# kwea123/nerf_pl

Hardware: AMD Instinct MI355X
Metric: rays/sec (64+128 samples), full training step: render_rays fwd + MSE + bwd + grad all-reduce + Adam (higher is better)
Workload: dtype bf16

## Files before the change

### nerf_pl_amd/csrc/mlp_bwd_dw.hip

```cpp
#include "mlp_device.h"
#include "mlp_bwd_dw.h"

namespace nerfhip {

#if NERFHIP_DW_PROBE
__device__ unsigned g_dw_probe[1024 * 8 * 8];
#endif

constexpr int kDwRingKiB = 160, kDwMaxDepth = 12;
constexpr int kDwFragRing = 5, kDwFragRing2D = 4;

template <int PREC> struct DwTraits;
template <> struct DwTraits<NERFHIP_BF16> {
    static constexpr int SPP = 1;
    static constexpr int RING_BYTES = kDwRingKiB * 1024;
    static constexpr int DEPTH = 0, STAGE_BYTES = 0;
};
template <> struct DwTraits<NERFHIP_F32> {
    static constexpr int SPP = 2;
    static constexpr int DEPTH = 2;
    static constexpr int MAXP = 72;
    static constexpr int STAGE_BYTES = MAXP * kPieceBytes;
    static constexpr int RING_BYTES = DEPTH * STAGE_BYTES;
};

template <int PREC> NH_HD constexpr int dw_depth(int pieces) {
    if (PREC != NERFHIP_BF16) return DwTraits<PREC>::DEPTH;
    const int d = DwTraits<PREC>::RING_BYTES / (pieces * kPieceBytes);
    return d > kDwMaxDepth ? kDwMaxDepth : d;
}

__device__ __forceinline__ void dw_bias_sum(const bf16x8& a, float& s0, float& s1) {
    const bf16x2 one = {(__bf16)1.0f, (__bf16)1.0f};
    s0 = __builtin_amdgcn_fdot2_f32_bf16(bf16x2{a[0], a[1]}, one, s0, false);
    s1 = __builtin_amdgcn_fdot2_f32_bf16(bf16x2{a[2], a[3]}, one, s1, false);
    s0 = __builtin_amdgcn_fdot2_f32_bf16(bf16x2{a[4], a[5]}, one, s0, false);
    s1 = __builtin_amdgcn_fdot2_f32_bf16(bf16x2{a[6], a[7]}, one, s1, false);
}

template <int F, int SLABS>
__device__ __forceinline__ bf16x8 dw_encode_slab(const float (&v)[3], int h, int ks) {
    constexpr int NPAIR = 3 * (F / 2);
    constexpr float kInv2PiHi = 0.15915494f, kInv2PiLo = 6.4206297e-9f;
    float rh[3], rl[3];
#pragma unroll
    for (int c = 0; c < 3; ++c) {
        const float vs = h ? 2.0f * v[c] : v[c];
        rh[c] = vs * kInv2PiHi;
        rl[c] = __builtin_fmaf(vs, kInv2PiHi, -rh[c]) + vs * kInv2PiLo;
    }
    bf16x8 out;
#pragma unroll
    for (int q = 0; q < 4; ++q) {
        const int p = 4 * ks + q;
        float s, co;
        if (p < NPAIR) {
            const int i = p / 3, c = p - 3 * i;
            const float sc = (float)(1 << (2 * i));
            const float rhc = c == 0 ? rh[0] : (c == 1 ? rh[1] : rh[2]), rlc = c == 0 ? rl[0] : (c == 1 ? rl[1] : rl[2]);
            const float t = __builtin_amdgcn_fractf(rhc * sc) + rlc * sc;
            s = __builtin_amdgcn_sinf(t);
            co = __builtin_amdgcn_cosf(t);
        } else {
            const int tail = 2 * (p - NPAIR);
            s = (tail == 0) ? (h ? v[2] : v[0]) : 0.0f;
            co = (tail == 0) ? (h ? 0.0f : v[1]) : 0.0f;
        }
        out[2 * q] = (__bf16)s;
        out[2 * q + 1] = (__bf16)co;
    }
    return out;
}

template <int PREC>
__global__ __launch_bounds__(512, 2)
void mlp_bwd_dw_kernel(DwJobTable jobs, float* __restrict__ slabs) {
    constexpr int SPP = DwTraits<PREC>::SPP;
    constexpr int SLAB_BYTES = SPP * kPieceBytes;
    constexpr int IL = act_il(PREC);
    constexpr int RING_BYTES = DwTraits<PREC>::RING_BYTES;
    __shared__ __attribute__((aligned(1024))) char ring[RING_BYTES];

    const int lane = threadIdx.x & 63;
    const int wave = __builtin_amdgcn_readfirstlane((int)(threadIdx.x >> 6));
    int jid = 0;
#pragma unroll
    for (int j = 1; j < kDwMaxJobs; ++j) jid += ((int)blockIdx.x >= jobs.soff[j]) ? 1 : 0;
    const int nsplit = jobs.nsplit[jid], split = (int)blockIdx.x - jobs.soff[jid];
    const DwJob jb = jobs.job[jid];
    const int64_t ntiles = jobs.ntiles[jid];
    const uint8_t* __restrict__ acts_base = jobs.acts[jid];
    const uint8_t* __restrict__ dys_base = jobs.dys[jid];
    [[maybe_unused]] const float* __restrict__ enc_rays = jobs.enc_rays[jid / kNumDwJobs];
    [[maybe_unused]] const float* __restrict__ enc_z = jobs.enc_z[jid / kNumDwJobs];
    [[maybe_unused]] const int enc_tpr = jobs.enc_tpr[jid / kNumDwJobs];
    const int n_ot = jb.dy_slabs / 2;
    const int n_xs = jb.x1_slabs + jb.x2_slabs;
    const int n_xt = n_xs / 2;
    const int64_t per = (ntiles + nsplit - 1) / nsplit;
    const int64_t t_first = (int64_t)split * per;
    const int64_t my_tiles = (t_first >= ntiles) ? 0 : ((ntiles - t_first < per) ? ntiles - t_first : per);
    const unsigned lds_base = (unsigned)(uintptr_t)ring;

    const int dma_off_even = (PREC == NERFHIP_BF16) ? ((lane & 1) * 32 + (lane >> 1)) * 16 : lane * 16;
    const int dma_off_odd = (PREC == NERFHIP_BF16) ? ((lane & 1) * 32 + ((lane ^ 8) >> 1)) * 16 : lane * 16;

    f32x16 acc[kDwMaxXTiles];
#pragma unroll
    for (int x = 0; x < kDwMaxXTiles; ++x)
#pragma unroll
        for (int r = 0; r < 16; ++r) acc[x][r] = 0.0f;
    float dbacc = 0.0f;
    [[maybe_unused]] float dbacc2 = 0.0f;

    const int grp = lane >> 4, c = lane & 15;
    const int tr_off = (grp & 1) * SLAB_BYTES + (2 * (8 * (grp >> 1) + (c >> 2)) + ((c & 3) & 1)) * 16 + ((c & 3) >> 1) * 8;
    const int tr_s0 = (grp & 1) ? 128 : 0, tr_s1 = 128 - tr_s0;
    [[maybe_unused]] auto load_frag = [&](const char* pb, int q) { return load_frag_tr16(pb, tr_off, tr_s0, tr_s1, q); };
    const int m32 = lane & 31, kk = lane >> 5;
    const int f32_off = (m32 >> 4) * SLAB_BYTES + (slab_nat_h(m32 & 15) * 32) * 32 + slab_nat_j(m32 & 15) * 4;
#if NERFHIP_DW_PROBE
    unsigned pr_wait = 0, pr_bar = 0, pr_issue = 0, pr_comp = 0, pr_depth = 0;
    const uint64_t pr_t00 = __builtin_amdgcn_s_memrealtime();
#endif

    auto run = [&](auto nxt_c, auto nsl_c, auto regen_c) {
        constexpr int NXT = decltype(nxt_c)::value, NSL = decltype(nsl_c)::value;
        constexpr bool REGEN = decltype(regen_c)::value;
        static_assert(!REGEN || (PREC == NERFHIP_BF16 && (NXT == 2 || NXT == 9 || NXT == 10)), "classes with an encoding section");
        constexpr int ENC = REGEN ? (NXT == 9 ? kDirSlabs : kXyzSlabs) : 0;
        constexpr int DYS = NXT == 9 ? 8 : 16;
        constexpr bool FOLD = NXT == 9 && NSL == kDwFoldStageSlabs;
        constexpr bool SPLIT2D = (PREC == NERFHIP_BF16) && (NXT == 8 || NXT == 10) && (NSL - 2 * NXT >= 16);
        constexpr int NP = NSL * SPP;
        constexpr int NPD = NP - ENC;
        constexpr int LPWD = (NPD + 7) / 8;
        constexpr int LPW = LPWD + (REGEN ? 1 : 0);
        constexpr int STAGE = (PREC == NERFHIP_BF16) ? NP * kPieceBytes : DwTraits<PREC>::STAGE_BYTES;
        constexpr int ZSLOT = 256;
        constexpr int D0 = dw_depth<PREC>(NP);
        constexpr int D = (REGEN && D0 * (STAGE + ZSLOT) > RING_BYTES) ? D0 - 1 : D0;
        static_assert(D >= 2 && D * (STAGE + (REGEN ? ZSLOT : 0)) <= RING_BYTES, "ring stages of this job class");
        static_assert((D - 2) * LPW <= 63, "counted vmcnt");
#if NERFHIP_DW_PROBE
        pr_depth = D;
#endif
        int s_issue = 0, s_use = 0;
        const uint8_t* abase = nullptr;
        const uint8_t* dbase = nullptr;
        unsigned slot = 0;
        auto stage_tile = [&](int64_t it) {
            int64_t T = t_first + (it < my_tiles ? it : my_tiles - 1);
            if (T >= ntiles) T = ntiles - 1;
            return T;
        };
        const float* zsrc = nullptr;
        unsigned zslot = 0;
        int z_issue = 0, g_slot = 0;
        const unsigned lds_z = lds_base + (unsigned)(D * STAGE);
        auto next_z = [&](int64_t st) {
            zsrc = enc_z + stage_tile(st) * 32 + (lane & 31);
            zslot = (unsigned)__builtin_amdgcn_readfirstlane((int)(lds_z + (unsigned)(z_issue * ZSLOT)));
            z_issue = (z_issue + 1 == D) ? 0 : z_issue + 1;
        };
        auto next_stage = [&](int64_t it) {
            const int64_t T = stage_tile(it);
            abase = acts_base + tile_block_off(T, act_tile_bytes(PREC), IL);
            dbase = dys_base + tile_block_off(T, kDySlabs * 64 * (16 * SPP), IL);
            slot = lds_base + (unsigned)(s_issue * STAGE);
            s_issue = (s_issue + 1 == D) ? 0 : s_issue + 1;
            if constexpr (REGEN) next_z(it + 1);
        };
        float ray_next[6] = {0.f, 0.f, 0.f, 0.f, 0.f, 0.f};
        auto load_ray = [&](int64_t st) {
            if (wave < ENC) {
                const unsigned r = (unsigned)__builtin_amdgcn_readfirstlane((int)((unsigned)stage_tile(st) / (unsigned)enc_tpr));
                typedef const float __attribute__((address_space(4))) * ConstF;
                const ConstF rp = (ConstF)(uintptr_t)(enc_rays + (size_t)r * 8);
#pragma unroll
                for (int c = 0; c < 6; ++c) ray_next[c] = rp[c];
            }
        };
        auto gen_stage = [&](int64_t st) {
            if (wave < ENC) {
                const int n = lane & 31, h = lane >> 5;
                bf16x8 e;
                if constexpr (NXT == 9) {
                    const float dv[3] = {ray_next[3], ray_next[4], ray_next[5]};
                    e = dw_encode_slab<4, kDirSlabs>(dv, h, wave);
                } else {
                    const float zv = *reinterpret_cast<const float*>(ring + D * STAGE + g_slot * ZSLOT + n * 4);
                    float xv[3];
#pragma unroll
                    for (int c = 0; c < 3; ++c) xv[c] = nh_add(ray_next[c], nh_mul(ray_next[3 + c], zv));
                    e = dw_encode_slab<10, kXyzSlabs>(xv, h, wave);
                }
                const int unit = (2 * n + h) ^ ((wave & 1) ? 8 : 0);
                *reinterpret_cast<bf16x8*>(ring + g_slot * STAGE + (DYS + wave) * SLAB_BYTES + unit * 16) = e;
            }
            g_slot = (g_slot + 1 == D) ? 0 : g_slot + 1;
            load_ray(st + 1);
        };
        constexpr int REM = NPD % 8;
        constexpr bool SHARE_LAST = (PREC == NERFHIP_BF16) && (REM == 4 || REM == 2);
        const int share_piece = NPD - REM + (SHARE_LAST ? (wave * REM) / 8 : 0);
        const unsigned long long share_mask = REM == 4 ? (0xffffffffull << (32 * (wave & 1))) : (0xffffull << (16 * (wave & 3)));
        auto issue_piece = [&](int i) {
            if constexpr (REGEN) {
                if (i == LPW - 1) {
                    glds4(zsrc, zslot);
                    return;
                }
            }
            int pi = wave + 8 * i;
            const bool shared = SHARE_LAST && i == LPWD - 1;
            if (shared) pi = share_piece;
            if (pi >= NPD) pi = NPD - 1;
            if (REGEN && pi >= DYS) pi += ENC;
            const int sl = pi / SPP, sub = pi % SPP;
            const uint8_t* src;
            if (FOLD && sl >= kDwFoldSigmaSlab) src = dbase + (size_t)(kDySigma + sl - kDwFoldSigmaSlab) * 64 * (16 * SPP) * IL;
            else if (sl < jb.dy_slabs) src = dbase + (size_t)(jb.dy_off + sl) * 64 * (16 * SPP) * IL;
            else if (sl < jb.dy_slabs + jb.x1_slabs) src = abase + (size_t)(jb.x1_off + sl - jb.dy_slabs) * 64 * (16 * SPP) * IL;
            else src = abase + (size_t)(jb.x2_off + sl - jb.dy_slabs - jb.x1_slabs) * 64 * (16 * SPP) * IL;
            const uint8_t* g = src + (size_t)sub * kPieceBytes + ((sl & 1) ? dma_off_odd : dma_off_even);
            const unsigned dst = (unsigned)__builtin_amdgcn_readfirstlane((int)(slot + (unsigned)(pi * kPieceBytes)));
            if (shared) glds16_nt_masked(g, dst, share_mask);
            else glds16_nt(g, dst);
        };
        auto issue_stage = [&](int64_t it) {
            next_stage(it);
#pragma unroll
            for (int i = 0; i < LPW; ++i) issue_piece(i);
        };
        constexpr bool SPREAD = (PREC == NERFHIP_BF16);
        constexpr int DMA_STEP = (2 * NXT) / LPW > 0 ? (2 * NXT) / LPW : 1;
        if constexpr (REGEN) {
            next_z(0);
            glds4(zsrc, zslot);
            load_ray(0);
        }
#pragma unroll
        for (int s = 0; s < D - 1; ++s) issue_stage(s);
        if constexpr (REGEN) {
            wait_vm<(D - 1) * LPW>();
            gen_stage(0);
        }
        for (int64_t it = 0; it < my_tiles; ++it) {
#if NERFHIP_DW_PROBE
            const unsigned t0 = shader_cycles();
            wait_vm<(PREC == NERFHIP_BF16) ? (D - 2) * LPW : 0>();
            const unsigned t1 = shader_cycles();
            asm volatile("s_barrier" ::: "memory");
            const unsigned t2 = shader_cycles();
            pr_wait += (t1 - t0) & 0xffffffffu;
            pr_bar += (t2 - t1) & 0xffffffffu;
#else
            wait_vm_barrier<(PREC == NERFHIP_BF16) ? (D - 2) * LPW : 0>();
#endif
            if (SPREAD && (SPLIT2D || wave < n_ot)) next_stage(it + D - 1);
            else issue_stage(it + D - 1);
#if NERFHIP_DW_PROBE
            const unsigned t3 = shader_cycles();
            pr_issue += (t3 - t2) & 0xffffffffu;
#endif
            const char* st_base = ring + s_use * STAGE;
            s_use = (s_use + 1 == D) ? 0 : s_use + 1;
            if constexpr (SPLIT2D) {
                constexpr int XW = NXT / 2, NF = 2 * XW, RD = kDwFragRing2D;
                static_assert(RD >= 2 && RD <= NF, "B fragment ring");
                const int wi = wave >> 1, wj = wave & 1;
                const char* dyb = st_base + (4 * wi) * SLAB_BYTES;
                const char* x_all = st_base + 16 * SLAB_BYTES;
                const char* xb = x_all + (2 * XW * wj) * SLAB_BYTES;
                auto dma_after = [](int k) constexpr { return ((k + 1) * NF) / LPW - 1; };
                bf16x8 a[2][2], b[RD];
                a[0][0] = load_frag(dyb, 0);
                a[0][1] = load_frag(dyb + 2 * SLAB_BYTES, 0);
#pragma unroll
                for (int f = 0; f < RD - 1; ++f) b[f] = load_frag(xb + 2 * (f % XW) * SLAB_BYTES, f / XW);
                a[1][0] = load_frag(dyb, 1);
                a[1][1] = load_frag(dyb + 2 * SLAB_BYTES, 1);
                __builtin_amdgcn_sched_barrier(0);
#pragma unroll
                for (int f = 0; f < NF; ++f) {
                    if (f + RD - 1 < NF) b[(f + RD - 1) % RD] = load_frag(xb + 2 * ((f + RD - 1) % XW) * SLAB_BYTES, (f + RD - 1) / XW);
                    __builtin_amdgcn_sched_barrier(0);
                    acc[2 * (f % XW)] = __builtin_amdgcn_mfma_f32_32x32x16_bf16(a[f / XW][0], b[f % RD], acc[2 * (f % XW)], 0, 0, 0);
                    acc[2 * (f % XW) + 1] = __builtin_amdgcn_mfma_f32_32x32x16_bf16(a[f / XW][1], b[f % RD], acc[2 * (f % XW) + 1], 0, 0, 0);
                    __builtin_amdgcn_sched_barrier(0);
                    if (f == 0 || f == XW) {
                        const bf16x8 ab = wj ? a[f / XW][1] : a[f / XW][0];
                        dw_bias_sum(ab, dbacc, dbacc2);
                    }
                    if constexpr (SPREAD) {
#pragma unroll
                        for (int k = 0; k < LPW; ++k)
                            if (dma_after(k) == f) {
                                issue_piece(k);
                                __builtin_amdgcn_sched_barrier(0);
                            }
                    }
                }
            } else if (wave < n_ot) {
                const char* dy_base = st_base + (2 * wave) * SLAB_BYTES;
                const char* x_base = st_base + jb.dy_slabs * SLAB_BYTES;
                if constexpr (PREC == NERFHIP_BF16) {
                    constexpr int RD = kDwFragRing, NM = 2 * NXT;
                    const bf16x8 a0 = load_frag(dy_base, 0);
                    bf16x8 b[RD];
#pragma unroll
                    for (int m = 0; m < RD - 1; ++m)
                        if (m < NM) b[m] = load_frag(x_base + 2 * (m % NXT) * SLAB_BYTES, m / NXT);
                    const bf16x8 a1 = load_frag(dy_base, 1);
                    __builtin_amdgcn_sched_barrier(0);
#pragma unroll
                    for (int m = 0; m < NM; ++m) {
                        const int x = m % NXT;
                        if (m + RD - 1 < NM) b[(m + RD - 1) % RD] = load_frag(x_base + 2 * ((m + RD - 1) % NXT) * SLAB_BYTES, (m + RD - 1) / NXT);
                        __builtin_amdgcn_sched_barrier(0);
                        acc[x] = __builtin_amdgcn_mfma_f32_32x32x16_bf16(m < NXT ? a0 : a1, b[m % RD], acc[x], 0, 0, 0);
                        __builtin_amdgcn_sched_barrier(0);
                        if (m == 1) dw_bias_sum(a0, dbacc, dbacc2);
                        if (m == NXT + 1 || (NXT == 1 && m == 1)) dw_bias_sum(a1, dbacc, dbacc2);
                        if constexpr (SPREAD) {
                            if (m % DMA_STEP == DMA_STEP - 1 && m / DMA_STEP < LPW) {
                                issue_piece(m / DMA_STEP);
                                __builtin_amdgcn_sched_barrier(0);
                            }
                        }
                    }
                    if constexpr (SPREAD) {
#pragma unroll
                        for (int i = (2 * NXT) / DMA_STEP; i < LPW; ++i) issue_piece(i);
                    }
                } else {
#pragma unroll 4
                    for (int ks = 0; ks < 16; ++ks) {
                        const int pt = 2 * ks + kk;
                        const float a = *reinterpret_cast<const float*>(dy_base + f32_off + pt * 32);
                        dbacc += a;
#pragma unroll
                        for (int x = 0; x < NXT; ++x) {
                            const float b = *reinterpret_cast<const float*>(x_base + 2 * x * SLAB_BYTES + f32_off + pt * 32);
                            acc[x] = __builtin_amdgcn_mfma_f32_32x32x2f32(a, b, acc[x], 0, 0, 0);
                        }
                    }
                }
            } else if constexpr (FOLD) {
                const char* sg = st_base + kDwFoldSigmaSlab * SLAB_BYTES;
                const char* xs = st_base + (jb.dy_slabs + 2 * (1 + 2 * (wave - kDwFoldRow0))) * SLAB_BYTES;
                if constexpr (PREC == NERFHIP_BF16) {
                    const bf16x8 a0 = load_frag(sg, 0), b00 = load_frag(xs, 0), b10 = load_frag(xs + 2 * SLAB_BYTES, 0);
                    const bf16x8 a1 = load_frag(sg, 1), b01 = load_frag(xs, 1), b11 = load_frag(xs + 2 * SLAB_BYTES, 1);
                    acc[0] = __builtin_amdgcn_mfma_f32_32x32x16_bf16(a0, b00, acc[0], 0, 0, 0);
                    acc[1] = __builtin_amdgcn_mfma_f32_32x32x16_bf16(a0, b10, acc[1], 0, 0, 0);
                    acc[0] = __builtin_amdgcn_mfma_f32_32x32x16_bf16(a1, b01, acc[0], 0, 0, 0);
                    acc[1] = __builtin_amdgcn_mfma_f32_32x32x16_bf16(a1, b11, acc[1], 0, 0, 0);
                    if (wave == kDwFoldRow0) {
                        dw_bias_sum(a0, dbacc, dbacc2);
                        dw_bias_sum(a1, dbacc, dbacc2);
                    }
                } else {
#pragma unroll 4
                    for (int ks = 0; ks < 16; ++ks) {
                        const int pt = 2 * ks + kk;
                        const float a = *reinterpret_cast<const float*>(sg + f32_off + pt * 32);
                        dbacc += a;
                        const float b0 = *reinterpret_cast<const float*>(xs + f32_off + pt * 32);
                        const float b1 = *reinterpret_cast<const float*>(xs + 2 * SLAB_BYTES + f32_off + pt * 32);
                        acc[0] = __builtin_amdgcn_mfma_f32_32x32x2f32(a, b0, acc[0], 0, 0, 0);
                        acc[1] = __builtin_amdgcn_mfma_f32_32x32x2f32(a, b1, acc[1], 0, 0, 0);
                    }
                }
            }
            if constexpr (REGEN) gen_stage(it + 1);
#if NERFHIP_DW_PROBE
            pr_comp += (shader_cycles() - t3) & 0xffffffffu;
#endif
        }
        asm volatile("s_waitcnt vmcnt(0)" ::: "memory");
        float* sl = slabs + (size_t)blockIdx.x * kDwSlabFloats;
        dbacc += dbacc2;
        if constexpr (SPLIT2D) {
            constexpr int XW = NXT / 2;
            const int wi = wave >> 1, wj = wave & 1;
#pragma unroll
            for (int xl = 0; xl < XW; ++xl)
#pragma unroll
                for (int d = 0; d < 2; ++d)
                    dw_store_block(sl + (size_t)((2 * wi + d) * kDwMaxXTiles + XW * wj + xl) * 1024, acc[2 * xl + d], lane);
            sl[8 * kDwMaxXTiles * 64 * 16 + (2 * wi + wj) * 64 + lane] = dbacc;
        } else if (wave < n_ot) {
#pragma unroll
            for (int x = 0; x < NXT; ++x) dw_store_block(sl + (size_t)(wave * kDwMaxXTiles + x) * 1024, acc[x], lane);
            sl[8 * kDwMaxXTiles * 64 * 16 + wave * 64 + lane] = dbacc;
        } else if constexpr (FOLD) {
            dw_store_block(sl + (size_t)dw_fold_block(2 * (wave - kDwFoldRow0)) * 1024, acc[0], lane);
            dw_store_block(sl + (size_t)dw_fold_block(2 * (wave - kDwFoldRow0) + 1) * 1024, acc[1], lane);
            if (wave == kDwFoldRow0) sl[8 * kDwMaxXTiles * 64 * 16 + kDwFoldRow0 * 64 + lane] = dbacc;
        }
    };
    using std::integral_constant;
    using std::false_type;
    using std::true_type;
    bool regen = false;
    if constexpr (PREC == NERFHIP_BF16) regen = enc_rays != nullptr;
    switch (n_xt) {
        case 2:
            if constexpr (PREC == NERFHIP_BF16) {
                if (regen) { run(integral_constant<int, 2>{}, integral_constant<int, 20>{}, true_type{}); break; }
            }
            run(integral_constant<int, 2>{}, integral_constant<int, 20>{}, false_type{});
            break;
        case 4: run(integral_constant<int, 4>{}, integral_constant<int, 10>{}, false_type{}); break;
        case 8:
            if (jb.dy_slabs == 16) run(integral_constant<int, 8>{}, integral_constant<int, 32>{}, false_type{});
            else run(integral_constant<int, 8>{}, integral_constant<int, 18>{}, false_type{});
            break;
        case 9:
            if (jobs.fold_of[(jid / kNumDwJobs) * kNumDwJobs + kDwJobSigma] == jid) {
                if constexpr (PREC == NERFHIP_BF16) {
                    if (regen) { run(integral_constant<int, 9>{}, integral_constant<int, kDwFoldStageSlabs>{}, true_type{}); break; }
                }
                run(integral_constant<int, 9>{}, integral_constant<int, kDwFoldStageSlabs>{}, false_type{});
            } else {
                run(integral_constant<int, 9>{}, integral_constant<int, 26>{}, false_type{});
            }
            break;
        default:
            if constexpr (PREC == NERFHIP_BF16) {
                if (regen) { run(integral_constant<int, 10>{}, integral_constant<int, 36>{}, true_type{}); break; }
            }
            run(integral_constant<int, 10>{}, integral_constant<int, 36>{}, false_type{});
            break;
    }
#if NERFHIP_DW_PROBE
    if (lane == 0 && blockIdx.x < 1024) {
        unsigned* pr = g_dw_probe + ((size_t)blockIdx.x * 8 + wave) * 8;
        pr[0] = (unsigned)my_tiles; pr[1] = pr_wait; pr[2] = pr_bar; pr[3] = pr_issue; pr[4] = pr_comp;
        pr[5] = (unsigned)(__builtin_amdgcn_s_memrealtime() - pr_t00);
        pr[6] = (unsigned)jid; pr[7] = pr_depth;
    }
#endif
}

NH_HD constexpr bool dw_job_has_class(const DwJob& j) {
    const int nxt = (j.x1_slabs + j.x2_slabs) / 2, nsl = j.dy_slabs + j.x1_slabs + j.x2_slabs;
    return (nxt == 2 && nsl == 20) || (nxt == 4 && nsl == 10) || (nxt == 8 && ((nsl == 32 && j.dy_slabs == 16) || (nsl == 18 && j.dy_slabs != 16))) ||
           (nxt == 9 && nsl == 26) || (nxt == 10 && nsl == 36);
}
NH_HD constexpr bool dw_jobs_have_classes() {
    for (int j = 0; j < kNumDwJobs; ++j)
        if (!dw_job_has_class(kDwJobs[j])) return false;
    return true;
}
static_assert(dw_jobs_have_classes(), "mlp_bwd_dw_kernel: a weight-gradient job without a compiled job class");

void launch_dw(int prec, const DwJobTable& jt, float* slabs, int nwg, hipStream_t s) {
    if (prec == NERFHIP_BF16) hipLaunchKernelGGL(mlp_bwd_dw_kernel<NERFHIP_BF16>, dim3(nwg), dim3(512), 0, s, jt, slabs);
    else hipLaunchKernelGGL(mlp_bwd_dw_kernel<NERFHIP_F32>, dim3(nwg), dim3(512), 0, s, jt, slabs);
}
#if NERFHIP_DW_PROBE
int read_dw_probe(unsigned* host_dst, int n_words) {
    return hipMemcpyFromSymbol(host_dst, HIP_SYMBOL(g_dw_probe), (size_t)n_words * 4, 0, hipMemcpyDeviceToHost) == hipSuccess ? 0 : -100;
}
#endif

}
```

Measured before the change: 1.095 million.

## Prefetch next tile's MFMA fragments across tile boundary and hoist DMA addressing

For bf16 non-regen job classes, the dW kernel now waits one stage further ahead and loads the first dY/X fragments of the next tile from LDS during the tail MFMAs of the current tile. This hides the LDS fragment-load latency at the tile boundary. It also precomputes per-piece global source pointers, LDS offsets and voffsets once, and issues the global-to-LDS loads through inline asm with scalar bases. This trims per-tile address arithmetic, but leaves one fewer stage in flight at the wait (requires D>=4) and raises register pressure.

```diff
diff --git a/nerf_pl_amd/csrc/mlp_bwd_dw.hip b/nerf_pl_amd/csrc/mlp_bwd_dw.hip
--- a/nerf_pl_amd/csrc/mlp_bwd_dw.hip
+++ b/nerf_pl_amd/csrc/mlp_bwd_dw.hip
@@ -72,6 +72,31 @@
     return out;
 }
 
+__device__ __forceinline__ size_t dw_uniform64(size_t v) {
+    size_t r;
+    asm("s_mov_b64 %0, %1" : "=s"(r) : "s"(v));
+    return r;
+}
+
+__device__ __forceinline__ void glds16_nt_sv(const void* sbase, unsigned voff, unsigned lds_dst) {
+    unsigned keep;
+    asm volatile(
+        "s_mov_b32 %0, m0\n\ts_mov_b32 m0, %3\n\ts_nop 0\n\tglobal_load_lds_dwordx4 %2, %1 nt\n\ts_mov_b32 m0, %0"
+        : "=&s"(keep)
+        : "s"(sbase), "v"(voff), "s"(lds_dst)
+        : "memory");
+}
+__device__ __forceinline__ void glds16_nt_sv_masked(const void* sbase, unsigned voff, unsigned lds_dst, unsigned long long mask) {
+    unsigned keep;
+    unsigned long long keep_exec;
+    asm volatile(
+        "s_mov_b32 %0, m0\n\ts_mov_b64 %1, exec\n\ts_mov_b32 m0, %4\n\ts_mov_b64 exec, %5\n\tglobal_load_lds_dwordx4 %3, %2 nt\n\t"
+        "s_mov_b64 exec, %1\n\ts_mov_b32 m0, %0"
+        : "=&s"(keep), "=&s"(keep_exec)
+        : "s"(sbase), "v"(voff), "s"(lds_dst), "s"(mask)
+        : "memory");
+}
+
 template <int PREC>
 __global__ __launch_bounds__(512, 2)
 void mlp_bwd_dw_kernel(DwJobTable jobs, float* __restrict__ slabs) {
@@ -142,6 +167,10 @@
         constexpr int D = (REGEN && D0 * (STAGE + ZSLOT) > RING_BYTES) ? D0 - 1 : D0;
         static_assert(D >= 2 && D * (STAGE + (REGEN ? ZSLOT : 0)) <= RING_BYTES, "ring stages of this job class");
         static_assert((D - 2) * LPW <= 63, "counted vmcnt");
+        constexpr bool AHEAD = (PREC == NERFHIP_BF16) && !REGEN;
+        constexpr bool HOIST = (PREC == NERFHIP_BF16) && !REGEN;
+        static_assert(!AHEAD || D >= 4, "certifying one stage ahead leaves D - 3 stages in flight at the wait");
+        constexpr int WAIT_N = (PREC == NERFHIP_BF16) ? (AHEAD ? D - 3 : D - 2) * LPW : 0;
 #if NERFHIP_DW_PROBE
         pr_depth = D;
 #endif
@@ -163,10 +192,16 @@
             zslot = (unsigned)__builtin_amdgcn_readfirstlane((int)(lds_z + (unsigned)(z_issue * ZSLOT)));
             z_issue = (z_issue + 1 == D) ? 0 : z_issue + 1;
         };
+        [[maybe_unused]] size_t a_delta = 0, d_delta = 0;
         auto next_stage = [&](int64_t it) {
             const int64_t T = stage_tile(it);
-            abase = acts_base + tile_block_off(T, act_tile_bytes(PREC), IL);
-            dbase = dys_base + tile_block_off(T, kDySlabs * 64 * (16 * SPP), IL);
+            if constexpr (HOIST) {
+                a_delta = dw_uniform64(tile_block_off(T, act_tile_bytes(PREC), IL));
+                d_delta = dw_uniform64(tile_block_off(T, kDySlabs * 64 * (16 * SPP), IL));
+            } else {
+                abase = acts_base + tile_block_off(T, act_tile_bytes(PREC), IL);
+                dbase = dys_base + tile_block_off(T, kDySlabs * 64 * (16 * SPP), IL);
+            }
             slot = lds_base + (unsigned)(s_issue * STAGE);
             s_issue = (s_issue + 1 == D) ? 0 : s_issue + 1;
             if constexpr (REGEN) next_z(it + 1);
@@ -205,7 +240,41 @@
         constexpr bool SHARE_LAST = (PREC == NERFHIP_BF16) && (REM == 4 || REM == 2);
         const int share_piece = NPD - REM + (SHARE_LAST ? (wave * REM) / 8 : 0);
         const unsigned long long share_mask = REM == 4 ? (0xffffffffull << (32 * (wave & 1))) : (0xffffull << (16 * (wave & 3)));
+        [[maybe_unused]] const uint8_t* pc_src[LPW];
+        [[maybe_unused]] bool pc_dy[LPW];
+        [[maybe_unused]] unsigned pc_lds[LPW];
+        [[maybe_unused]] unsigned pc_voff = 0, pc_voff_last = 0;
+        if constexpr (HOIST) {
+#pragma unroll
+            for (int i = 0; i < LPW; ++i) {
+                int pi = wave + 8 * i;
+                if (i == LPW - 1) {
+                    if (SHARE_LAST) pi = share_piece;
+                    if (pi >= NPD) pi = NPD - 1;
+                }
+                const int sl = pi;
+                const bool dy = (FOLD && sl >= kDwFoldSigmaSlab) || sl < jb.dy_slabs;
+                int gs;
+                if (FOLD && sl >= kDwFoldSigmaSlab) gs = kDySigma + sl - kDwFoldSigmaSlab;
+                else if (sl < jb.dy_slabs) gs = jb.dy_off + sl;
+                else if (sl < jb.dy_slabs + jb.x1_slabs) gs = jb.x1_off + sl - jb.dy_slabs;
+                else gs = jb.x2_off + sl - jb.dy_slabs - jb.x1_slabs;
+                pc_dy[i] = __builtin_amdgcn_readfirstlane((int)dy) != 0;
+                pc_src[i] = (dy ? dys_base : acts_base) + (size_t)__builtin_amdgcn_readfirstlane(gs) * 64 * 16 * IL;
+                pc_lds[i] = (unsigned)__builtin_amdgcn_readfirstlane(pi * kPieceBytes);
+                const unsigned voff = (unsigned)((sl & 1) ? dma_off_odd : dma_off_even);
+                if (i == LPW - 1) pc_voff_last = voff;
+                else pc_voff = voff;
+            }
+        }
         auto issue_piece = [&](int i) {
+            if constexpr (HOIST) {
+                const uint8_t* src = pc_src[i] + (pc_dy[i] ? d_delta : a_delta);
+                const unsigned dst = slot + pc_lds[i];
+                if (SHARE_LAST && i == LPW - 1) glds16_nt_sv_masked(src, pc_voff_last, dst, share_mask);
+                else glds16_nt_sv(src, i == LPW - 1 ? pc_voff_last : pc_voff, dst);
+                return;
+            }
             if constexpr (REGEN) {
                 if (i == LPW - 1) {
                     glds4(zsrc, zslot);
@@ -246,17 +315,41 @@
             wait_vm<(D - 1) * LPW>();
             gen_stage(0);
         }
+        constexpr int NB = SPLIT2D ? NXT : 2 * NXT;
+        constexpr int RDC = SPLIT2D ? (NB % 4 == 0 ? 4 : 5) : (NB % 6 == 0 ? 6 : 4);
+        static_assert(!AHEAD || (NB % RDC == 0 && RDC - 1 <= NB), "the B ring's slots must come round at the tile boundary");
+        [[maybe_unused]] bf16x8 ca[2], cb[RDC];
+        [[maybe_unused]] auto carry_a = [&](const char* sb) {
+            if constexpr (SPLIT2D) {
+                ca[0] = load_frag(sb + (4 * (wave >> 1)) * SLAB_BYTES, 0);
+                ca[1] = load_frag(sb + (4 * (wave >> 1) + 2) * SLAB_BYTES, 0);
+            } else {
+                ca[0] = load_frag(sb + (2 * wave) * SLAB_BYTES, 0);
+            }
+        };
+        [[maybe_unused]] auto carry_b = [&](const char* sb, int f) {
+            if constexpr (SPLIT2D) cb[f] = load_frag(sb + (16 + NXT * (wave & 1) + 2 * (f % (NXT / 2))) * SLAB_BYTES, f / (NXT / 2));
+            else cb[f] = load_frag(sb + (jb.dy_slabs + 2 * (f % NXT)) * SLAB_BYTES, f / NXT);
+        };
+        if constexpr (AHEAD) {
+            wait_vm_barrier<WAIT_N>();
+            if (SPLIT2D || wave < n_ot) {
+                carry_a(ring);
+#pragma unroll
+                for (int f = 0; f < RDC - 1; ++f) carry_b(ring, f);
+            }
+        }
         for (int64_t it = 0; it < my_tiles; ++it) {
 #if NERFHIP_DW_PROBE
             const unsigned t0 = shader_cycles();
-            wait_vm<(PREC == NERFHIP_BF16) ? (D - 2) * LPW : 0>();
+            wait_vm<WAIT_N>();
             const unsigned t1 = shader_cycles();
             asm volatile("s_barrier" ::: "memory");
             const unsigned t2 = shader_cycles();
             pr_wait += (t1 - t0) & 0xffffffffu;
             pr_bar += (t2 - t1) & 0xffffffffu;
 #else
-            wait_vm_barrier<(PREC == NERFHIP_BF16) ? (D - 2) * LPW : 0>();
+            wait_vm_barrier<WAIT_N>();
 #endif
             if (SPREAD && (SPLIT2D || wave < n_ot)) next_stage(it + D - 1);
             else issue_stage(it + D - 1);
@@ -266,7 +359,38 @@
 #endif
             const char* st_base = ring + s_use * STAGE;
             s_use = (s_use + 1 == D) ? 0 : s_use + 1;
-            if constexpr (SPLIT2D) {
+            [[maybe_unused]] const char* nx_base = ring + s_use * STAGE;
+            if constexpr (SPLIT2D && AHEAD) {
+                constexpr int XW = NXT / 2, NF = 2 * XW, RD = RDC;
+                constexpr int CA_AT = (NF - (RD - 1) > XW) ? NF - (RD - 1) : XW;
+                const int wi = wave >> 1, wj = wave & 1;
+                const char* dyb = st_base + (4 * wi) * SLAB_BYTES;
+                const char* xb = st_base + (16 + 2 * XW * wj) * SLAB_BYTES;
+                auto dma_after = [](int k) constexpr { return ((k + 1) * NF) / LPW - 1; };
+                bf16x8 a1[2];
+#pragma unroll
+                for (int f = 0; f < NF; ++f) {
+                    if (f == CA_AT) carry_a(nx_base);
+                    if (f == 1) {
+                        a1[0] = load_frag(dyb, 1);
+                        a1[1] = load_frag(dyb + 2 * SLAB_BYTES, 1);
+                    }
+                    if (f + RD - 1 < NF) cb[(f + RD - 1) % RD] = load_frag(xb + 2 * ((f + RD - 1) % XW) * SLAB_BYTES, (f + RD - 1) / XW);
+                    else carry_b(nx_base, f + RD - 1 - NF);
+                    __builtin_amdgcn_sched_barrier(0);
+                    acc[2 * (f % XW)] = __builtin_amdgcn_mfma_f32_32x32x16_bf16(f < XW ? ca[0] : a1[0], cb[f % RD], acc[2 * (f % XW)], 0, 0, 0);
+                    acc[2 * (f % XW) + 1] = __builtin_amdgcn_mfma_f32_32x32x16_bf16(f < XW ? ca[1] : a1[1], cb[f % RD], acc[2 * (f % XW) + 1], 0, 0, 0);
+                    __builtin_amdgcn_sched_barrier(0);
+                    if (f == 0) dw_bias_sum(wj ? ca[1] : ca[0], dbacc, dbacc2);
+                    if (f == XW) dw_bias_sum(wj ? a1[1] : a1[0], dbacc, dbacc2);
+#pragma unroll
+                    for (int k = 0; k < LPW; ++k)
+                        if (dma_after(k) == f) {
+                            issue_piece(k);
+                            __builtin_amdgcn_sched_barrier(0);
+                        }
+                }
+            } else if constexpr (SPLIT2D) {
                 constexpr int XW = NXT / 2, NF = 2 * XW, RD = kDwFragRing2D;
                 static_assert(RD >= 2 && RD <= NF, "B fragment ring");
                 const int wi = wave >> 1, wj = wave & 1;
@@ -305,7 +429,32 @@
             } else if (wave < n_ot) {
                 const char* dy_base = st_base + (2 * wave) * SLAB_BYTES;
                 const char* x_base = st_base + jb.dy_slabs * SLAB_BYTES;
-                if constexpr (PREC == NERFHIP_BF16) {
+                if constexpr (AHEAD) {
+                    constexpr int RD = RDC, NM = 2 * NXT;
+                    constexpr int CA_LO = NXT > 2 ? NXT : 2;
+                    constexpr int CA_AT = (NM - (RD - 1) > CA_LO) ? NM - (RD - 1) : CA_LO;
+                    static_assert(CA_AT < NM, "a step of this tile to carry the next dY fragment under");
+                    bf16x8 a1;
+#pragma unroll
+                    for (int m = 0; m < NM; ++m) {
+                        const int x = m % NXT;
+                        if (m == CA_AT) carry_a(nx_base);
+                        if (m == 1) a1 = load_frag(dy_base, 1);
+                        if (m + RD - 1 < NM) cb[(m + RD - 1) % RD] = load_frag(x_base + 2 * ((m + RD - 1) % NXT) * SLAB_BYTES, (m + RD - 1) / NXT);
+                        else carry_b(nx_base, m + RD - 1 - NM);
+                        __builtin_amdgcn_sched_barrier(0);
+                        acc[x] = __builtin_amdgcn_mfma_f32_32x32x16_bf16(m < NXT ? ca[0] : a1, cb[m % RD], acc[x], 0, 0, 0);
+                        __builtin_amdgcn_sched_barrier(0);
+                        if (m == 1) dw_bias_sum(ca[0], dbacc, dbacc2);
+                        if (m == NXT + 1) dw_bias_sum(a1, dbacc, dbacc2);
+                        if (m % DMA_STEP == DMA_STEP - 1 && m / DMA_STEP < LPW) {
+                            issue_piece(m / DMA_STEP);
+                            __builtin_amdgcn_sched_barrier(0);
+                        }
+                    }
+#pragma unroll
+                    for (int i = (2 * NXT) / DMA_STEP; i < LPW; ++i) issue_piece(i);
+                } else if constexpr (PREC == NERFHIP_BF16) {
                     constexpr int RD = kDwFragRing, NM = 2 * NXT;
                     const bf16x8 a0 = load_frag(dy_base, 0);
                     bf16x8 b[RD];
```

After: 1.101 million, median of 6. About the same (+0.5%).
